# cvigilv/SimSpread.jl

Measured on AMD Instinct MI355X. Metric: predicted edges/sec + achieved HBM GB/s, W*R SpMM, higher is better.
Workload: dtype f32

## Files before the change

simspread.jl_amd/csrc/transfer.hip:

```cpp
#include <type_traits>

#include "graph.hpp"

namespace ss {

template <class T>
struct ChunkedView {
  const int* off;
  const unsigned short* idx;
  const T* val;
  int64_t rows;
};
template <class T>
static inline ChunkedView<T> view(const DevChunked<T>& m) {
  return ChunkedView<T>{m.off.p, m.idx.p, m.val.p, m.rows};
}

template <class T>
struct TransferArgs {
  int nterms;
  CsrView<T> L[2];
  const T* inv1[2];
  ChunkedView<T> M[2];
  const T* inv2;
  const int* kf;
  const int* ks;
  int64_t row_begin;
  const int* row_ids;
  int64_t nj;
  int SC;
  int nchunks;
  T* out;
  int64_t ld;
  int accumulate;
  float xmax;
  int chunk_interleave;
};
template <class T>
__device__ __forceinline__ bool chunks_in_turn(const TransferArgs<T>& p) { return p.chunk_interleave != 0; }

template <class F>
static int dispatch_bool(bool b, F&& f) {
  return b ? f(std::true_type{}) : f(std::false_type{});
}
template <int... Vs, class F>
static int dispatch_int(int v, F&& f) {
  int rc = SS_OK;
  const bool hit = ((v == Vs && ((rc = f(std::integral_constant<int, Vs>{})), true)) || ...);
  return hit ? rc : fail(SS_EINVAL, "dispatch_int: no kernel for the value %d", v);
}

template <auto Kernel, class... Args>
static int launch_lds(unsigned grid, int block, size_t lds, Args... args) {
  static std::atomic<bool> attr_done{false};
  if (!attr_done) {
    SS_HIP(hipFuncSetAttribute(reinterpret_cast<const void*>(Kernel), hipFuncAttributeMaxDynamicSharedMemorySize,
                               160 * 1024));
    attr_done = true;
  }
  hipLaunchKernelGGL(Kernel, dim3(grid), dim3(block), lds, ctx().stream, args...);
  SS_LAUNCH_CHECK();
  return SS_OK;
}

constexpr int TRANSFER_THREADS = 64;

template <class T> struct BitsOf;
template <> struct BitsOf<float> {
  static __device__ __forceinline__ float bcast(float v, int src) {
    return __int_as_float(__builtin_amdgcn_readlane(__float_as_int(v), src));
  }
  static __device__ __forceinline__ float push(int to4, float v) {
    return __int_as_float(__builtin_amdgcn_ds_permute(to4, __float_as_int(v)));
  }
  static __device__ __forceinline__ float pull(int from4, float v) {
    return __int_as_float(__builtin_amdgcn_ds_bpermute(from4, __float_as_int(v)));
  }
};
template <> struct BitsOf<double> {
  static __device__ __forceinline__ double join(int lo, int hi) {
    return __longlong_as_double(((long long)hi << 32) | (unsigned int)lo);
  }
  static __device__ __forceinline__ double bcast(double v, int src) {
    const long long b = __double_as_longlong(v);
    const int lo = __builtin_amdgcn_readlane((int)(b & 0xffffffffll), src);
    const int hi = __builtin_amdgcn_readlane((int)(b >> 32), src);
    return join(lo, hi);
  }
  static __device__ __forceinline__ double push(int to4, double v) {
    const long long b = __double_as_longlong(v);
    return join(__builtin_amdgcn_ds_permute(to4, (int)(b & 0xffffffffll)), __builtin_amdgcn_ds_permute(to4, (int)(b >> 32)));
  }
  static __device__ __forceinline__ double pull(int from4, double v) {
    const long long b = __double_as_longlong(v);
    return join(__builtin_amdgcn_ds_bpermute(from4, (int)(b & 0xffffffffll)), __builtin_amdgcn_ds_bpermute(from4, (int)(b >> 32)));
  }
};

template <class T, int U>
struct SubRows {
  int n[U];
  unsigned b[U];
  T cf[U];
  unsigned short j[U];
  T v[U];
};

template <int U, bool BINM>
__device__ __forceinline__ void subrows_load_buf(SubRows<float, U>& s, int first, int b_l, int n_l, float cf_l,
                                                 __amdgpu_buffer_rsrc_t ridx, __amdgpu_buffer_rsrc_t rval, int lane) {
#pragma unroll
  for (int u = 0; u < U; ++u) {
    const int src = first + u;
    s.b[u] = (unsigned)__builtin_amdgcn_readlane(b_l, src);
    s.n[u] = __builtin_amdgcn_readlane(n_l, src);
    s.cf[u] = BitsOf<float>::bcast(cf_l, src);
    s.j[u] = __builtin_amdgcn_raw_buffer_load_b16(ridx, lane * 2, (int)(s.b[u] * 2u), 0);
    s.v[u] = BINM ? 1.f : __builtin_bit_cast(float, __builtin_amdgcn_raw_buffer_load_b32(rval, lane * 4, (int)(s.b[u] * 4u), 0));
    __builtin_amdgcn_sched_barrier(0);
  }
}

template <class T, int U, bool BINM>
__device__ __forceinline__ void subrows_load(SubRows<T, U>& s, int first, int b_l, int n_l, T cf_l,
                                             const unsigned short* __restrict__ midx, const T* __restrict__ mval,
                                             int lane) {
#pragma unroll
  for (int u = 0; u < U; ++u) {
    const int src = first + u;
    s.b[u] = (unsigned)__builtin_amdgcn_readlane(b_l, src);
    s.n[u] = __builtin_amdgcn_readlane(n_l, src);
    s.cf[u] = BitsOf<T>::bcast(cf_l, src);
    const unsigned short* pi = midx + s.b[u];
    const T* pv = mval + s.b[u];
    s.j[u] = pi[lane];
    s.v[u] = BINM ? T(1) : pv[lane];
    __builtin_amdgcn_sched_barrier(0);
  }
}

template <class T, int U, bool DUAL>
__device__ __forceinline__ void subrows_fold(const SubRows<T, U>& s, T* __restrict__ acc, int astride, int dummy, int lane) {
  if constexpr (DUAL) {
    T* __restrict__ acc1 = acc + astride;
#pragma unroll
    for (int u = 0; u < U; u += 2) {
      const int ja = lane < s.n[u] ? (int)s.j[u] : dummy;
      const int jb = lane < s.n[u + 1] ? (int)s.j[u + 1] : dummy;
      const T ra = acc[ja], rb = acc1[jb];
      acc[ja] = fma(s.cf[u], s.v[u], ra);
      acc1[jb] = fma(s.cf[u + 1], s.v[u + 1], rb);
    }
  } else {
#pragma unroll
    for (int u = 0; u < U; ++u) {
      const int j = lane < s.n[u] ? (int)s.j[u] : dummy;
      acc[j] = fma(s.cf[u], s.v[u], acc[j]);
    }
  }
}

__device__ __forceinline__ int cvt_rpi(float x) {
  int r;
  asm("v_cvt_rpi_i32_f32 %0, %1" : "=v"(r) : "v"(x));
  return r;
}
template <int U>
__device__ __forceinline__ void subrows_fold_fixed(const SubRows<float, U>& s, unsigned* __restrict__ acc, int lane) {
#pragma unroll
  for (int u = 0; u < U; ++u) {
    const float v = lane < s.n[u] ? s.v[u] : 0.f;
    atomicAdd(&acc[s.j[u]], (unsigned)cvt_rpi(s.cf[u] * v));
  }
}

template <class T, int U, bool DUAL, bool FIX>
__device__ __forceinline__ void subrows_fold_any(const SubRows<T, U>& s, T* acc, int astride, int dummy, int lane) {
  if constexpr (FIX) subrows_fold_fixed<U>(s, reinterpret_cast<unsigned*>(acc), lane);
  else subrows_fold<T, U, DUAL>(s, acc, astride, dummy, lane);
}

template <class T, int AHEAD>
struct Tails {
  static constexpr int TAIL_AHEAD = AHEAD;
  int nt;
  int cb, cn;
  T ccf;
  unsigned short tj[TAIL_AHEAD];
  T tv[TAIL_AHEAD];
};

template <class T, int TAIL_AHEAD, class LD>
__device__ __forceinline__ void tails_fetch(Tails<T, TAIL_AHEAD>& t, int r0, int lane, LD&& ld) {
#pragma unroll
  for (int i = 0; i < TAIL_AHEAD; ++i) {
    if (4 * (r0 + i) >= t.nt) break;
    const unsigned b = (unsigned)__builtin_amdgcn_ds_bpermute((4 * (r0 + i) + (lane >> 4)) * 4, t.cb);
    ld(b + 64u + (unsigned)(lane & 15), t.tj[i], t.tv[i]);
    __builtin_amdgcn_sched_barrier(0);
  }
}

template <class T, int TAIL_AHEAD, class LD>
__device__ __forceinline__ void tails_begin(Tails<T, TAIL_AHEAD>& t, int b_l, int n_l, T cf_l, int lane, LD&& ld) {
  const unsigned long long longs = __ballot(n_l > 64);
  t.nt = __builtin_popcountll(longs);
  if (t.nt == 0) return;
  const int k = (int)__builtin_amdgcn_mbcnt_hi((unsigned)(longs >> 32), __builtin_amdgcn_mbcnt_lo((unsigned)longs, 0u));
  const int to4 = (n_l > 64 ? k : t.nt + lane - k) * 4;
  t.cb = __builtin_amdgcn_ds_permute(to4, b_l);
  t.cn = __builtin_amdgcn_ds_permute(to4, n_l);
  t.ccf = BitsOf<T>::push(to4, cf_l);
  tails_fetch(t, 0, lane, ld);
}

template <class T, bool BINM, bool FIX, int TAIL_AHEAD, class LD>
__device__ __forceinline__ void tails_finish(Tails<T, TAIL_AHEAD>& t, int b_l, int n_l, T cf_l, T* __restrict__ acc, int dummy,
                                             const unsigned short* __restrict__ midx, const T* __restrict__ mval, int lane,
                                             LD&& ld) {
  if (t.nt == 0) return;
  for (int r0 = 0; 4 * r0 < t.nt; r0 += TAIL_AHEAD) {
    if (r0 > 0) tails_fetch(t, r0, lane, ld);
#pragma unroll
    for (int i = 0; i < TAIL_AHEAD; ++i) {
      if (4 * (r0 + i) >= t.nt) break;
      const int from4 = (4 * (r0 + i) + (lane >> 4)) * 4;
      const int tn = __builtin_amdgcn_ds_bpermute(from4, t.cn) - 64;
      const T tcf = BitsOf<T>::pull(from4, t.ccf);
      const bool live = (lane & 15) < tn;
      if constexpr (FIX) {
        atomicAdd(reinterpret_cast<unsigned*>(acc) + (live ? (int)t.tj[i] : dummy),
                  (unsigned)cvt_rpi(live ? (float)(tcf * t.tv[i]) : 0.f));
      } else {
#pragma unroll
        for (int g = 0; g < 4; ++g) {
          const int j = (live && (lane >> 4) == g) ? (int)t.tj[i] : dummy;
          acc[j] = fma(tcf, t.tv[i], acc[j]);
        }
      }
    }
  }
  unsigned long long m = __ballot(n_l > 80);
  while (m != 0ull) {
    const int src = __builtin_ctzll(m);
    m &= m - 1ull;
    const int n = __builtin_amdgcn_readlane(n_l, src);
    const unsigned b = (unsigned)__builtin_amdgcn_readlane(b_l, src);
    const T cf = BitsOf<T>::bcast(cf_l, src);
    for (int x = 80 + lane; x < n; x += 64) {
      const int j = midx[b + x];
      const T v = BINM ? T(1) : mval[b + x];
      if constexpr (FIX) atomicAdd(reinterpret_cast<unsigned*>(acc) + j, (unsigned)cvt_rpi((float)(cf * v)));
      else acc[j] = fma(cf, v, acc[j]);
    }
  }
}

struct FixedScale {
  float scale, unscale;
};
template <class F>
__device__ __forceinline__ FixedScale fixed_scale(int lb, int le, int lane, float xmax, F&& abs_coef) {
  float sabs = 0.f;
  for (int q = lb + lane; q < le; q += 64) sabs += abs_coef(q);
#pragma unroll
  for (int o = 32; o > 0; o >>= 1) sabs += __shfl_xor(sabs, o);
  int e = 0;
  (void)frexpf(sabs * xmax, &e);
  if (!(sabs * xmax > 0.f)) e = 0;
  e = e < -90 ? -90 : (e > 120 ? 120 : e);
  return FixedScale{ldexpf(1.f, 30 - e), ldexpf(1.f, e - 30)};
}

template <class T, bool LOO, int U, bool BINM, bool DUAL, bool FIX = false, bool BUF = false>
__global__ void __launch_bounds__(TRANSFER_THREADS) transfer_kernel(TransferArgs<T> p) {
  static_assert(64 % (2 * U) == 0, "U must divide 32");
  extern __shared__ __align__(16) unsigned char smem_raw[];
  T* acc = reinterpret_cast<T*>(smem_raw);
  const int astride = p.SC + 64;
  constexpr int NCOPY = DUAL ? 2 : 1;
  unsigned* bits = reinterpret_cast<unsigned*>(acc + NCOPY * astride);
  const int lane = threadIdx.x;
  int c;
  int64_t r;
  if (p.nchunks > 8 && p.nchunks % 8 == 0 && !chunks_in_turn(p)) {
    const int64_t nrows = (int64_t)gridDim.x / p.nchunks, per = nrows * 8;
    const int64_t grp = blockIdx.x / per, rem = blockIdx.x - grp * per;
    r = rem >> 3;
    c = (int)(grp * 8 + (rem & 7));
  } else {
    c = blockIdx.x % p.nchunks;
    r = blockIdx.x / p.nchunks;
  }
  const int64_t gr = p.row_ids ? (int64_t)p.row_ids[p.row_begin + r] : p.row_begin + r;
  const int64_t j0 = (int64_t)c * p.SC;
  const int jn = (int)((p.nj - j0 < p.SC) ? (p.nj - j0) : p.SC);
  const int dummy = p.SC + lane;

  for (int j = lane; j < NCOPY * astride; j += 64) acc[j] = T(0);
  if (LOO)
    for (int j = lane; j < (p.SC + 31) / 32; j += 64) bits[j] = 0u;
  __syncthreads();

  float fix_unscale = 1.f;
  for (int t = 0; t < p.nterms; ++t) {
    const CsrView<T> L = p.L[t];
    const ChunkedView<T> M = p.M[t];
    const int* __restrict__ off = M.off + (int64_t)c * M.rows;
    const unsigned short* __restrict__ midx = M.idx;
    const T* __restrict__ mval = M.val;
    const int lb = L.ptr[gr], le = L.ptr[gr + 1];
    float scale = 1.f;
    if constexpr (FIX) {
      float sabs = 0.f;
      for (int q = lb + lane; q < le; q += 64) sabs += fabsf((float)(L.val[q] * p.inv1[t][L.idx[q]]));
#pragma unroll
      for (int o = 32; o > 0; o >>= 1) sabs += __shfl_xor(sabs, o);
      int e = 0;
      (void)frexpf(sabs * p.xmax, &e);
      if (!(sabs * p.xmax > 0.f)) e = 0;
      e = e < -90 ? -90 : (e > 120 ? 120 : e);
      scale = ldexpf(1.f, 30 - e);
      fix_unscale = ldexpf(1.f, e - 30);
    }
    for (int g0 = lb; g0 < le; g0 += 64) {
      const int q = g0 + lane;
      int b_l = 0, n_l = 0;
      T cf_l = T(0);
      if (q < le) {
        const int a = L.idx[q];
        const T lv = L.val[q];
        if (LOO) {
          const int d = p.kf[a] - 1;
          cf_l = (a != (int)gr && d > 0) ? lv * (T(1) / T(d)) : T(0);
        } else {
          cf_l = lv * p.inv1[t][a];
          if constexpr (FIX) cf_l = (T)((float)cf_l * scale);
        }
        if (cf_l != T(0)) { b_l = off[a]; n_l = off[a + 1] - b_l; }
      }
      const int cnt = __builtin_amdgcn_readfirstlane((le - g0 < 64) ? (le - g0) : 64);
      SubRows<T, U> A, B;
      auto load = [&](SubRows<T, U>& sr, int first) __attribute__((always_inline)) {
        if constexpr (BUF) {
          const __amdgpu_buffer_rsrc_t ridx = __builtin_amdgcn_make_buffer_rsrc((void*)midx, 0, -1, 0x00020000);
          const __amdgpu_buffer_rsrc_t rval = __builtin_amdgcn_make_buffer_rsrc((void*)mval, 0, -1, 0x00020000);
          subrows_load_buf<U, BINM>(sr, first, b_l, n_l, cf_l, ridx, rval, lane);
        } else {
          subrows_load<T, U, BINM>(sr, first, b_l, n_l, cf_l, midx, mval, lane);
        }
      };
      auto tail_ld = [&](unsigned e, unsigned short& j, T& v) __attribute__((always_inline)) {
        if constexpr (BUF) {
          const __amdgpu_buffer_rsrc_t ridx = __builtin_amdgcn_make_buffer_rsrc((void*)midx, 0, -1, 0x00020000);
          const __amdgpu_buffer_rsrc_t rval = __builtin_amdgcn_make_buffer_rsrc((void*)mval, 0, -1, 0x00020000);
          j = __builtin_amdgcn_raw_buffer_load_b16(ridx, (int)(e * 2u), 0, 0);
          v = BINM ? 1.f : __builtin_bit_cast(float, __builtin_amdgcn_raw_buffer_load_b32(rval, (int)(e * 4u), 0, 0));
        } else {
          j = midx[e];
          v = BINM ? T(1) : mval[e];
        }
      };
      Tails<T, (BINM ? 4 : 2)> tails;
      tails_begin(tails, b_l, n_l, cf_l, lane, tail_ld);
      load(A, 0);
      for (int u0 = 0; u0 < cnt; u0 += 2 * U) {
        if (u0 + U < cnt) load(B, u0 + U);
        subrows_fold_any<T, U, DUAL, FIX>(A, acc, astride, dummy, lane);
        if (u0 + U < cnt) {
          if (u0 + 2 * U < cnt) load(A, u0 + 2 * U);
          subrows_fold_any<T, U, DUAL, FIX>(B, acc, astride, dummy, lane);
        }
      }
      tails_finish<T, BINM, FIX>(tails, b_l, n_l, cf_l, acc, dummy, midx, mval, lane, tail_ld);
    }
  }
  if (LOO) {
    const ChunkedView<T> M = p.M[0];
    const int* off = M.off + (int64_t)c * M.rows;
    for (int x = off[gr] + lane; x < off[gr + 1]; x += 64) {
      const int j = M.idx[x];
      atomicOr(&bits[j >> 5], 1u << (j & 31));
    }
  }
  __syncthreads();

  T* orow = p.out + r * p.ld + j0;
  for (int j = lane; j < jn; j += 64) {
    T z;
    T sum = DUAL ? acc[j] + acc[astride + j] : acc[j];
    if constexpr (FIX) sum = (T)((float)reinterpret_cast<const int*>(acc)[j] * fix_unscale);
    if (LOO) {
      const int d = p.ks[j0 + j] - (int)((bits[j >> 5] >> (j & 31)) & 1u);
      z = (d > 0 && (j0 + j) != gr) ? sum * (T(1) / T(d)) : T(0);
    } else {
      z = sum * p.inv2[j0 + j];
      if (p.accumulate) z += orow[j];
    }
    orow[j] = z;
  }
}

constexpr int TRANSFER_U = 8;

static bool transfer_dual() { return env_int("SS_TRANSFER_DUAL", 0) != 0; }

static int transfer_u() {
  const int u = (int)env_int("SS_TRANSFER_U", TRANSFER_U);
  return (u == 4 || u == 16) ? u : 8;
}

template <class T>
__global__ void transfer_coef_kernel(const int* __restrict__ ptr, const int* __restrict__ idx, const T* __restrict__ val,
                                     const T* __restrict__ inv1, int64_t row_begin, int64_t nrows, T* __restrict__ coef) {
  const int lo = ptr[row_begin], hi = ptr[row_begin + nrows];
  for (int64_t e = (int64_t)lo + (int64_t)blockIdx.x * blockDim.x + threadIdx.x; e < hi; e += (int64_t)gridDim.x * blockDim.x)
    coef[e] = val[e] * inv1[idx[e]];
}

enum { TB_PLAIN, TB_QFLAT, TB_WIDE, TB_WIDE2 };
constexpr int WIDE_META = 64 * 12;
constexpr int WIDE_LIST = 64;
constexpr int W2_TBL = 64 * 12;
template <int KIND, class T>
struct BlockLayout {
  static constexpr bool EXACT = KIND != TB_PLAIN;
  static constexpr int shared_bytes = KIND == TB_WIDE ? 64 : 0;
  __host__ __device__ static int64_t offs_bytes(int64_t mrows) { return (((mrows + 1) * 4 + 15) / 16) * 16; }
  __host__ __device__ static int64_t lens_bytes(int64_t mrows) { return EXACT ? ((mrows * 2 + 15) / 16) * 16 : 0; }
  __host__ __device__ static int acc_elems(int SC) { return SC + 64; }
  __host__ __device__ static int acc_bytes(int SC) {
    return KIND == TB_WIDE || KIND == TB_WIDE2 ? (((SC + 4) * 4 + 15) / 16) * 16 : acc_elems(SC) * (int)sizeof(T);
  }
  __host__ __device__ static int per_wave(int SC) {
    return acc_bytes(SC) + (KIND == TB_WIDE ? WIDE_META + WIDE_LIST : KIND == TB_WIDE2 ? 2 * W2_TBL + 4 * 64 : 0);
  }
  __device__ static unsigned char* wave_base(unsigned char* smem, int offs_b, int lens_b, int wave, int SC) {
    return smem + offs_b + lens_b + shared_bytes + (size_t)wave * (size_t)per_wave(SC);
  }
};

struct BlockWave {
  int lane, c, jn, lb, le;
  int64_t r, gr, j0;
};

template <bool EXACT, class T, class A>
__device__ __forceinline__ bool block_prologue(BlockWave& w, const TransferArgs<T>& p, int64_t nrows, int wave, int* offs,
                                               unsigned short* lens, const unsigned short* glen, A* acc, int nacc) {
  const int nw = blockDim.x >> 6;
  w.lane = threadIdx.x & 63;
  w.c = blockIdx.x % p.nchunks;
  w.r = (int64_t)(blockIdx.x / p.nchunks) * nw + wave;
  const ChunkedView<T> M = p.M[0];
  {
    const int* __restrict__ off = M.off + (int64_t)w.c * M.rows;
    for (int64_t i = threadIdx.x; i <= M.rows; i += blockDim.x) offs[i] = off[i];
    if constexpr (EXACT) {
      const unsigned short* __restrict__ gl = glen + (int64_t)w.c * M.rows;
      for (int64_t i = threadIdx.x; i < M.rows; i += blockDim.x) lens[i] = gl[i];
    }
  }
  for (int j = w.lane; j < nacc; j += 64) acc[j] = A(0);
  __syncthreads();
  return w.r < nrows;
}
template <class T>
__device__ __forceinline__ void block_row(BlockWave& w, const TransferArgs<T>& p) {
  w.gr = p.row_begin + w.r;
  w.j0 = (int64_t)w.c * p.SC;
  w.jn = (int)((p.nj - w.j0 < p.SC) ? (p.nj - w.j0) : p.SC);
  const int* lptr = p.L[0].ptr;
  w.lb = __builtin_amdgcn_readfirstlane(lptr[w.gr]);
  w.le = __builtin_amdgcn_readfirstlane(lptr[w.gr + 1]);
}

template <class T>
__device__ __forceinline__ void fixed_store(const TransferArgs<T>& p, int64_t r, int64_t j0, int jn, int lane, const void* acc,
                                            float unscale) {
  T* orow = p.out + r * p.ld + j0;
  const int* iacc = reinterpret_cast<const int*>(acc);
  for (int j = lane; j < jn; j += 64) orow[j] = (T)((float)iacc[j] * unscale) * p.inv2[j0 + j];
}

typedef float f4 __attribute__((ext_vector_type(4)));
typedef unsigned u2 __attribute__((ext_vector_type(2)));

template <bool BINM>
__device__ __forceinline__ void quad_fetch(const u2* midx4, const f4* mval4, int quad, float cfv, int rem, u2& oj, f4& ov,
                                           float& ocf) {
  ocf = cfv;
  oj = midx4[quad];
  if constexpr (BINM) ov = f4{rem > 0 ? 1.f : 0.f, rem > 1 ? 1.f : 0.f, rem > 2 ? 1.f : 0.f, rem > 3 ? 1.f : 0.f};
  else ov = mval4[quad];
}
__device__ __forceinline__ void quad_fold(unsigned* acc, u2 j, f4 v, float cf) {
  atomicAdd(acc + (j.x & 0xffffu), (unsigned)cvt_rpi(cf * v.x));
  atomicAdd(acc + (j.x >> 16), (unsigned)cvt_rpi(cf * v.y));
  atomicAdd(acc + (j.y & 0xffffu), (unsigned)cvt_rpi(cf * v.z));
  atomicAdd(acc + (j.y >> 16), (unsigned)cvt_rpi(cf * v.w));
}

__device__ __forceinline__ void raw_load(const int* lidx, const float* coef, int lb, int le, int lane, int g, int& a, float& cf) {
  const int q = lb + g * 64 + lane;
  a = 0;
  cf = 0.f;
  if (q < le) { a = lidx[q]; cf = coef[q]; }
}

template <class T, int U, bool BINM, bool FIX>
__global__ void __launch_bounds__(1024) transfer_block_kernel(TransferArgs<T> p, const T* __restrict__ coef, int64_t nrows,
                                                              int align, int offs_bytes, float xmax) {
  using Lay = BlockLayout<TB_PLAIN, T>;
  extern __shared__ __align__(16) unsigned char smem_raw[];
  int* offs = reinterpret_cast<int*>(smem_raw);
  const int wave = threadIdx.x >> 6;
  const int astride = p.SC + 64;
  T* acc = reinterpret_cast<T*>(smem_raw + offs_bytes) + (size_t)wave * Lay::acc_elems(p.SC);
  BlockWave w;
  if (!block_prologue<false>(w, p, nrows, wave, offs, nullptr, nullptr, acc, astride)) return;
  w.gr = p.row_begin + w.r;
  w.j0 = (int64_t)w.c * p.SC;
  w.jn = (int)((p.nj - w.j0 < p.SC) ? (p.nj - w.j0) : p.SC);
  const int lane = w.lane, lb = p.L[0].ptr[w.gr], le = p.L[0].ptr[w.gr + 1];
  const int dummy = p.SC + lane;
  const CsrView<T> L = p.L[0];
  const unsigned short* __restrict__ midx = p.M[0].idx;
  const T* __restrict__ mval = p.M[0].val;
  float scale = 1.f, unscale = 1.f;
  if constexpr (FIX) {
    const FixedScale fs = fixed_scale(lb, le, lane, xmax, [&](int q) __attribute__((always_inline)) { return fabsf((float)coef[q]); });
    scale = fs.scale;
    unscale = fs.unscale;
  }
  for (int g0 = lb; g0 < le; g0 += 64) {
    const int q = g0 + lane;
    int b_l = 0, n_l = 0;
    T cf_l = T(0);
    if (q < le) {
      const int a = L.idx[q];
      cf_l = coef[q];
      if constexpr (FIX) cf_l = (T)((float)cf_l * scale);
      if (cf_l != T(0)) {
        const int o0 = offs[a], o1 = offs[a + 1];
        b_l = o0 * align;
        n_l = (o1 - o0) * align;
      }
    }
    const int cnt = __builtin_amdgcn_readfirstlane((le - g0 < 64) ? (le - g0) : 64);
    SubRows<T, U> A, B;
    auto load = [&](SubRows<T, U>& sr, int first) __attribute__((always_inline)) {
      subrows_load<T, U, BINM>(sr, first, b_l, n_l, cf_l, midx, mval, lane);
    };
    auto tail_ld = [&](unsigned e, unsigned short& j, T& v) __attribute__((always_inline)) {
      j = midx[e];
      v = BINM ? T(1) : mval[e];
    };
    Tails<T, (BINM ? 4 : 2)> tails;
    tails_begin(tails, b_l, n_l, cf_l, lane, tail_ld);
    load(A, 0);
    for (int u0 = 0; u0 < cnt; u0 += 2 * U) {
      if (u0 + U < cnt) load(B, u0 + U);
      subrows_fold_any<T, U, false, FIX>(A, acc, astride, dummy, lane);
      if (u0 + U < cnt) {
        if (u0 + 2 * U < cnt) load(A, u0 + 2 * U);
        subrows_fold_any<T, U, false, FIX>(B, acc, astride, dummy, lane);
      }
    }
    tails_finish<T, BINM, FIX>(tails, b_l, n_l, cf_l, acc, dummy, midx, mval, lane, tail_ld);
  }
  if constexpr (FIX) {
    fixed_store(p, w.r, w.j0, w.jn, lane, acc, unscale);
  } else {
    T* orow = p.out + w.r * p.ld + w.j0;
    for (int j = lane; j < w.jn; j += 64) orow[j] = acc[j] * p.inv2[w.j0 + j];
  }
}

template <class T, int D, bool BINM>
__global__ void __launch_bounds__(1024) transfer_qflat_kernel(TransferArgs<T> p, const T* __restrict__ coef, int64_t nrows,
                                                             int align, int offs_bytes, int lens_bytes, float xmax,
                                                             const unsigned short* __restrict__ glen) {
  static_assert(std::is_same<T, float>::value, "fixed-point sums: fp32 graphs only");
  extern __shared__ __align__(16) unsigned char smem_raw[];
  int* offs = reinterpret_cast<int*>(smem_raw);
  unsigned short* lens = reinterpret_cast<unsigned short*>(smem_raw + offs_bytes);
  const int lane = threadIdx.x & 63;
  const int wave = __builtin_amdgcn_readfirstlane(threadIdx.x >> 6);
  const int astride = p.SC + 64;
  unsigned* acc = reinterpret_cast<unsigned*>(BlockLayout<TB_QFLAT, T>::wave_base(smem_raw, offs_bytes, lens_bytes, wave, p.SC));
  BlockWave w;
  if (!block_prologue<true>(w, p, nrows, wave, offs, lens, glen, acc, astride)) return;
  block_row(w, p);
  const ChunkedView<T> M = p.M[0];
  const CsrView<T> L = p.L[0];
  const int64_t r = w.r, j0 = w.j0;
  const int jn = w.jn, lb = w.lb, le = w.le;
  const unsigned short* __restrict__ midx = M.idx;
  const T* __restrict__ mval = M.val;
  float scale, unscale;
  {
    float sabs = 0.f;
    for (int q = lb + lane; q < le; q += 64) sabs += fabsf(coef[q]);
#pragma unroll
    for (int o = 32; o > 0; o >>= 1) sabs += __shfl_xor(sabs, o);
    int e = 0;
    (void)frexpf(sabs * xmax, &e);
    if (!(sabs * xmax > 0.f)) e = 0;
    e = e < -90 ? -90 : (e > 120 ? 120 : e);
    scale = ldexpf(1.f, 30 - e);
    unscale = ldexpf(1.f, e - 30);
  }
  const int ngroups = (le - lb + 63) >> 6;
  auto raw_load = [&](int g, int& a, float& cf) __attribute__((always_inline)) {
    const int q = lb + g * 64 + lane;
    a = 0;
    cf = 0.f;
    if (q < le) { a = L.idx[q]; cf = coef[q]; }
  };
  auto meta = [&](int a, float cf, int& b_l, int& n_l, float& cf_l) __attribute__((always_inline)) {
    cf_l = cf * scale;
    b_l = 0;
    n_l = 0;
    if (cf_l != 0.f) {
      b_l = (offs[a] * align) >> 2;
      n_l = ((int)lens[a] + 3) >> 2;
    }
  };
  int Pc = 0, dc = 0, ra, bn, nn;
  float cc = 0.f, cn, rc;
  int total = 0, nst = 0, t = 0, gcur = -1;
  raw_load(0, ra, rc); meta(ra, rc, bn, nn, cn);
  raw_load(1, ra, rc);
  bool done = false;
  auto switch_group = [&]() __attribute__((always_inline)) {
    ++gcur;
    int incl = nn;
#pragma unroll
    for (int o = 1; o < 64; o <<= 1) {
      const int up = __shfl_up(incl, o);
      if (lane >= o) incl += up;
    }
    Pc = incl - nn;
    dc = bn - Pc;
    cc = cn;
    total = __builtin_amdgcn_readlane(incl, 63);
    nst = (total + 63) >> 6;
    t = 0;
    meta(ra, rc, bn, nn, cn);
    raw_load(gcur + 2, ra, rc);
  };
  u2 sj[D];
  f4 sv[D];
  float sc[D];
  const f4* __restrict__ mval4 = reinterpret_cast<const f4*>(mval);
  const u2* __restrict__ midx4 = reinterpret_cast<const u2*>(midx);
  auto next_step = [&](u2& oj, f4& ov, float& ocf) __attribute__((always_inline)) {
    if (t >= nst) {
      if (gcur + 1 < ngroups) switch_group();
      else done = true;
    }
    float cfv = 0.f;
    int addr = lane;
    if (t < nst) {
      const int lo = t << 6;
      const int pos = lo + lane;
      const unsigned long long le_mask = __ballot(Pc <= lo);
      const int own0 = __builtin_popcountll(le_mask) - 1;
      unsigned long long m = __ballot(Pc > lo && Pc <= lo + 63);
      cfv = __int_as_float(__builtin_amdgcn_readlane(__float_as_int(cc), own0));
      int dlv = __builtin_amdgcn_readlane(dc, own0);
      while (m != 0ull) {
        const int i = __builtin_ctzll(m);
        m &= m - 1ull;
        const int Pi = __builtin_amdgcn_readlane(Pc, i);
        const float cfi = __int_as_float(__builtin_amdgcn_readlane(__float_as_int(cc), i));
        const int dli = __builtin_amdgcn_readlane(dc, i);
        const bool in = pos >= Pi;
        cfv = in ? cfi : cfv;
        dlv = in ? dli : dlv;
      }
      const bool valid = pos < total;
      cfv = valid ? cfv : 0.f;
      addr = valid ? pos + dlv : lane;
      ++t;
    }
    quad_fetch<BINM>(midx4, mval4, addr, cfv, 4, oj, ov, ocf);
  };
#pragma unroll
  for (int i = 0; i < D; ++i) next_step(sj[i], sv[i], sc[i]);
  while (!done) {
#pragma unroll
    for (int i = 0; i < D; ++i) {
      quad_fold(acc, sj[i], sv[i], sc[i]);
      next_step(sj[i], sv[i], sc[i]);
    }
  }
#pragma unroll
  for (int i = 0; i < D; ++i) quad_fold(acc, sj[i], sv[i], sc[i]);
  fixed_store(p, r, j0, jn, lane, acc, unscale);
}

template <int D, bool BINM>
__global__ void __launch_bounds__(1024) transfer_wide_kernel(TransferArgs<float> p, const float* __restrict__ coef,
                                                             int64_t nrows, int align, int offs_bytes, int lens_bytes,
                                                             float xmax, const unsigned short* __restrict__ glen) {
  extern __shared__ __align__(16) unsigned char smem_raw[];
  int* offs = reinterpret_cast<int*>(smem_raw);
  unsigned short* lens = reinterpret_cast<unsigned short*>(smem_raw + offs_bytes);
  unsigned char* ident = smem_raw + offs_bytes + lens_bytes;
  const int lane = threadIdx.x & 63, nw = blockDim.x >> 6;
  const int wave = __builtin_amdgcn_readfirstlane(threadIdx.x >> 6);
  using Lay = BlockLayout<TB_WIDE, float>;
  const int accb = Lay::acc_bytes(p.SC);
  unsigned char* mine = Lay::wave_base(smem_raw, offs_bytes, lens_bytes, wave, p.SC);
  unsigned* acc = reinterpret_cast<unsigned*>(mine);
  unsigned char* metab = mine + accb;
  unsigned char* list = metab + WIDE_META;
  const int c = blockIdx.x % p.nchunks;
  const int64_t r = (int64_t)(blockIdx.x / p.nchunks) * nw + wave;
  const ChunkedView<float> M = p.M[0];
  const CsrView<float> L = p.L[0];
  {
    const int* __restrict__ off = M.off + (int64_t)c * M.rows;
    const unsigned short* __restrict__ gl = glen + (int64_t)c * M.rows;
    for (int64_t i = threadIdx.x; i <= M.rows; i += blockDim.x) offs[i] = off[i];
    for (int64_t i = threadIdx.x; i < M.rows; i += blockDim.x) lens[i] = gl[i];
    if (threadIdx.x < 64) ident[threadIdx.x] = (unsigned char)threadIdx.x;
  }
  for (int j = lane; j < p.SC; j += 64) acc[j] = 0u;
  __syncthreads();
  if (r >= nrows) return;
  const int64_t gr = p.row_begin + r;
  const int64_t j0 = (int64_t)c * p.SC;
  const int jn = (int)((p.nj - j0 < p.SC) ? (p.nj - j0) : p.SC);
  const int lb = __builtin_amdgcn_readfirstlane(L.ptr[gr]), le = __builtin_amdgcn_readfirstlane(L.ptr[gr + 1]);
  const FixedScale fs = fixed_scale(lb, le, lane, xmax, [&](int q) __attribute__((always_inline)) { return fabsf(coef[q]); });
  const float scale = fs.scale, unscale = fs.unscale;
  const int ngroups = (le - lb + 63) >> 6;
  const f4* __restrict__ mval4 = reinterpret_cast<const f4*>(M.val);
  const u2* __restrict__ midx4 = reinterpret_cast<const u2*>(M.idx);
  int gcur = -1, level = 0, st = 0, nst = 0, nlist = 0, qoff = 0;
  int ncur = 0;
  int ra;
  float rc;
  raw_load(L.idx, coef, lb, le, lane, 0, ra, rc);
  bool done = false;
  auto open_group = [&]() __attribute__((always_inline)) {
    ++gcur;
    const float cf = rc * scale;
    int b = 0, n = 0;
    if (cf != 0.f) { b = (offs[ra] * align) >> 2; n = (int)lens[ra]; }
    raw_load(L.idx, coef, lb, le, lane, gcur + 1, ra, rc);
    ncur = n;
    unsigned* m = reinterpret_cast<unsigned*>(metab + lane * 12);
    m[0] = (unsigned)b; m[1] = (unsigned)n; m[2] = __float_as_uint(cf);
    level = 0;
    st = 0;
    qoff = 0;
    const int cnt = (le - lb - gcur * 64 < 64) ? (le - lb - gcur * 64) : 64;
    nlist = cnt;
    nst = (cnt + 3) >> 2;
  };
  auto next_level = [&]() __attribute__((always_inline)) {
    const int covered = 64 + 16 * level;
    ++level;
    qoff = covered >> 2;
    const bool more = ncur > covered;
    const unsigned long long mk = __ballot(more);
    nlist = __builtin_popcountll(mk);
    if (more) list[__builtin_amdgcn_mbcnt_hi((unsigned)(mk >> 32), __builtin_amdgcn_mbcnt_lo((unsigned)mk, 0u))] = (unsigned char)lane;
    st = 0;
    nst = (nlist + 15) >> 4;
  };
  u2 sj[D];
  f4 sv[D];
  float sc[D];
  auto next_step = [&](u2& oj, f4& ov, float& ocf) __attribute__((always_inline)) {
    if (st >= nst) {
      if (gcur >= 0 && nlist > 0) next_level();
      else if (gcur + 1 < ngroups) open_group();
      else done = true;
    }
    float cfv = 0.f;
    int quad = lane;
    int rem = 0;
    if (st < nst) {
      const int sh = level == 0 ? 4 : 2;
      const int pos = (st << (6 - sh)) + (lane >> sh);
      const int e = lane & ((1 << sh) - 1);
      const unsigned char* lst = level == 0 ? ident : list;
      const int fi = pos < nlist ? (int)lst[pos] : 0;
      const unsigned* m = reinterpret_cast<const unsigned*>(metab + fi * 12);
      const int b = (int)m[0], n = (int)m[1];
      const float cf = __uint_as_float(m[2]);
      const int qe = qoff + e;
      const bool valid = pos < nlist && 4 * qe < n;
      cfv = valid ? cf : 0.f;
      quad = valid ? b + qe : lane;
      rem = n - 4 * qe;
      ++st;
    }
    quad_fetch<BINM>(midx4, mval4, quad, cfv, rem, oj, ov, ocf);
  };
#pragma unroll
  for (int i = 0; i < D; ++i) next_step(sj[i], sv[i], sc[i]);
  while (!done) {
#pragma unroll
    for (int i = 0; i < D; ++i) {
      quad_fold(acc, sj[i], sv[i], sc[i]);
      next_step(sj[i], sv[i], sc[i]);
    }
  }
#pragma unroll
  for (int i = 0; i < D; ++i) quad_fold(acc, sj[i], sv[i], sc[i]);
  float* orow = p.out + r * p.ld + j0;
  const int* iacc = reinterpret_cast<const int*>(acc);
  for (int j = lane; j < jn; j += 64) orow[j] = ((float)iacc[j] * unscale) * p.inv2[j0 + j];
}

constexpr int W2_STEPS = 20;
constexpr int W2_D = 4;
template <bool BINM>
__global__ void __launch_bounds__(1024) transfer_wide2_kernel(TransferArgs<float> p, const float* __restrict__ coef,
                                                              int64_t nrows, int align, int offs_bytes, int lens_bytes,
                                                              float xmax, const unsigned short* __restrict__ glen) {
  extern __shared__ __align__(16) unsigned char smem_raw[];
  int* offs = reinterpret_cast<int*>(smem_raw);
  unsigned short* lens = reinterpret_cast<unsigned short*>(smem_raw + offs_bytes);
  const int lane = threadIdx.x & 63, nw = blockDim.x >> 6;
  const int wave = __builtin_amdgcn_readfirstlane(threadIdx.x >> 6);
  using Lay = BlockLayout<TB_WIDE2, float>;
  const int accb = Lay::acc_bytes(p.SC);
  unsigned char* mine = Lay::wave_base(smem_raw, offs_bytes, lens_bytes, wave, p.SC);
  unsigned* acc = reinterpret_cast<unsigned*>(mine);
  unsigned char* tbl0 = mine + accb;
  unsigned char* lst0 = tbl0 + 2 * W2_TBL;
  const int c = blockIdx.x % p.nchunks;
  const int64_t r = (int64_t)(blockIdx.x / p.nchunks) * nw + wave;
  const ChunkedView<float> M = p.M[0];
  const CsrView<float> L = p.L[0];
  {
    const int* __restrict__ off = M.off + (int64_t)c * M.rows;
    const unsigned short* __restrict__ gl = glen + (int64_t)c * M.rows;
    for (int64_t i = threadIdx.x; i <= M.rows; i += blockDim.x) offs[i] = off[i];
    for (int64_t i = threadIdx.x; i < M.rows; i += blockDim.x) lens[i] = gl[i];
  }
  for (int j = lane; j < p.SC; j += 64) acc[j] = 0u;
  __syncthreads();
  if (r >= nrows) return;
  const int64_t gr = p.row_begin + r;
  const int64_t j0 = (int64_t)c * p.SC;
  const int jn = (int)((p.nj - j0 < p.SC) ? (p.nj - j0) : p.SC);
  const int lb = __builtin_amdgcn_readfirstlane(L.ptr[gr]), le = __builtin_amdgcn_readfirstlane(L.ptr[gr + 1]);
  const FixedScale fs = fixed_scale(lb, le, lane, xmax, [&](int q) __attribute__((always_inline)) { return fabsf(coef[q]); });
  const float scale = fs.scale, unscale = fs.unscale;
  const int ngroups = (le - lb + 63) >> 6;
  const f4* __restrict__ mval4 = reinterpret_cast<const f4*>(M.val);
  const u2* __restrict__ midx4 = reinterpret_cast<const u2*>(M.idx);
  const unsigned short* __restrict__ midx = M.idx;
  const float* __restrict__ mval = M.val;
  const int lastq = le > lb ? le - 1 : lb;
  auto raw_load = [&](int g, int& a, float& cf) __attribute__((always_inline)) {
    const int q = lb + g * 64 + lane;
    const int qc = q < le ? q : lastq;
    a = L.idx[qc];
    const float x = coef[qc];
    cf = q < le ? x : 0.f;
  };
  int ra = 0;
  float rc = 0.f;
  auto open_group = [&](int g) __attribute__((always_inline)) {
    unsigned char* tb = tbl0 + (g & 1) * W2_TBL;
    unsigned char* l1 = lst0 + (g & 1) * 128;
    unsigned char* l2 = l1 + 64;
    const float cf = (g < ngroups) ? rc * scale : 0.f;
    int b = 0, n = 0;
    if (cf != 0.f) { b = (offs[ra] * align) >> 2; n = (int)lens[ra]; }
    raw_load(g + 1, ra, rc);
    unsigned* m = reinterpret_cast<unsigned*>(tb + lane * 12);
    m[0] = (unsigned)b; m[1] = (unsigned)n; m[2] = __float_as_uint(cf);
    const unsigned long long m1 = __ballot(n > 64);
    const int r1 = __builtin_amdgcn_mbcnt_hi((unsigned)(m1 >> 32), __builtin_amdgcn_mbcnt_lo((unsigned)m1, 0u));
    const bool in1 = n > 64 && r1 < 48;
    const unsigned long long m2 = __ballot(in1 && n > 80);
    const int r2 = __builtin_amdgcn_mbcnt_hi((unsigned)(m2 >> 32), __builtin_amdgcn_mbcnt_lo((unsigned)m2, 0u));
    const bool in2 = in1 && n > 80 && r2 < 16;
    l1[lane] = 255; l2[lane] = 255;
    if (in1) l1[r1] = (unsigned char)lane;
    if (in2) l2[r2] = (unsigned char)lane;
    const int cov = in2 ? 96 : (in1 ? 80 : 64);
    if (__ballot(n > cov) != 0ull) {
      for (int x = cov; x < n; ++x) {
        const int at = 4 * b + x;
        atomicAdd(acc + midx[at], (unsigned)cvt_rpi(cf * (BINM ? 1.f : mval[at])));
      }
    }
  };
  u2 sj[W2_D];
  f4 sv[W2_D];
  float sc[W2_D];
  auto gen = [&](int s, int par, u2& oj, f4& ov, float& ocf) __attribute__((always_inline)) {
    const unsigned char* tb = tbl0 + par * W2_TBL;
    int fi, e, qoff;
    bool have = true;
    if (s < 16) {
      fi = 4 * s + (lane >> 4);
      e = lane & 15;
      qoff = 0;
    } else {
      const unsigned char* lst = lst0 + par * 128 + (s < 19 ? 0 : 64);
      const int pos = (s < 19 ? 16 * (s - 16) : 0) + (lane >> 2);
      fi = (int)lst[pos];
      have = fi != 255;
      fi = have ? fi : 0;
      e = lane & 3;
      qoff = s < 19 ? 16 : 20;
    }
    const unsigned* m = reinterpret_cast<const unsigned*>(tb + fi * 12);
    const int b = (int)m[0], n = (int)m[1];
    const float cf = __uint_as_float(m[2]);
    const int qe = qoff + e;
    const bool valid = have && 4 * qe < n;
    quad_fetch<BINM>(midx4, mval4, valid ? b + qe : lane, valid ? cf : 0.f, n - 4 * qe, oj, ov, ocf);
  };
  if (ngroups > 0) {
    raw_load(0, ra, rc);
    open_group(0);
#pragma unroll
    for (int i = 0; i < W2_D; ++i) gen(i, 0, sj[i], sv[i], sc[i]);
    for (int g = 0; g < ngroups; ++g) {
      const int par = g & 1;
#pragma unroll
      for (int s = 0; s < W2_STEPS; ++s) {
        if (s == W2_STEPS - W2_D) open_group(g + 1);
        quad_fold(acc, sj[s % W2_D], sv[s % W2_D], sc[s % W2_D]);
        if (s + W2_D < W2_STEPS) gen(s + W2_D, par, sj[s % W2_D], sv[s % W2_D], sc[s % W2_D]);
        else gen(s + W2_D - W2_STEPS, par ^ 1, sj[s % W2_D], sv[s % W2_D], sc[s % W2_D]);
      }
    }
  }
  fixed_store(p, r, j0, jn, lane, acc, unscale);
}

template <int KIND, class T>
static int transfer_block_waves(int64_t mrows, int SC) {
  using Lay = BlockLayout<KIND, T>;
  const int64_t fixed_bytes = Lay::offs_bytes(mrows) + Lay::lens_bytes(mrows) + Lay::shared_bytes;
  const int64_t room = (int64_t)ctx().lds_per_block - fixed_bytes;
  int64_t nw = room > 0 ? room / Lay::per_wave(SC) : 0;
  if (nw > 16) nw = 16;
  nw = env_int_in("SS_TRANSFER_NW", 1, nw, nw);
  return nw >= 8 ? (int)nw : 0;
}

template <class T>
bool transfer_block_fits(int64_t mrows, int SC) {
  return transfer_block_waves<TB_PLAIN, T>(mrows, SC) > 0;
}

template <int KIND, auto Kernel, class T>
static int launch_block_kernel(const TransferArgs<T>& p, const DevChunked<T>& Mt, const T* coef, int64_t nrows, int nw,
                               float xmax) {
  using Lay = BlockLayout<KIND, T>;
  const int offs_bytes = (int)Lay::offs_bytes(Mt.rows), lens_bytes = (int)Lay::lens_bytes(Mt.rows);
  const unsigned grid = (unsigned)(ceil_div(nrows, (int64_t)nw) * p.nchunks);
  const size_t lds = (size_t)offs_bytes + (size_t)lens_bytes + Lay::shared_bytes + (size_t)nw * (size_t)Lay::per_wave(p.SC);
  if constexpr (Lay::EXACT)
    return launch_lds<Kernel>(grid, 64 * nw, lds, p, coef, nrows, Mt.align, offs_bytes, lens_bytes, xmax,
                              (const unsigned short*)Mt.len.p);
  else
    return launch_lds<Kernel>(grid, 64 * nw, lds, p, coef, nrows, Mt.align, offs_bytes, xmax);
}

template <class T>
int launch_transfer_block(const DevCsr<T>& L, const T* inv1, const DevChunked<T>& Mt, const T* inv2, int64_t row_begin,
                          int64_t nrows, int64_t nj, T* out, int64_t ld, T* coef, float xmax, bool fixed) {
  if (nrows <= 0 || nj <= 0) return SS_OK;
  const int nw = transfer_block_waves<TB_PLAIN, T>(Mt.rows, Mt.SC);
  if (nw == 0) return fail(SS_EUNSUPPORTED, "transfer_block: offsets + accumulators do not fit in LDS");
  TransferArgs<T> p{};
  p.nterms = 1;
  p.L[0] = view(L);
  p.M[0] = view(Mt);
  p.inv2 = inv2;
  p.row_begin = row_begin;
  p.nj = nj;
  p.SC = Mt.SC;
  p.nchunks = Mt.nchunks;
  p.out = out;
  p.ld = ld;
  if (ceil_div(nrows, (int64_t)nw) * p.nchunks >= (1LL << 31))
    return fail(SS_EUNSUPPORTED, "transfer grid too large; lower SS_TRANSFER_BYTES");
  path_add("transfer_block");
  hipLaunchKernelGGL(transfer_coef_kernel<T>, dim3(grid_1d(L.nnz > 0 ? L.nnz : 1, 256, 256 * 8)), dim3(256), 0, ctx().stream,
                     L.ptr.p, L.idx.p, L.val.p, inv1, row_begin, nrows, coef);
  SS_LAUNCH_CHECK();
  constexpr bool CANFIX = std::is_same<T, float>::value;
  const bool fx = CANFIX && fixed;
  if (fx) path_add("fixed_point");
  const bool binm = Mt.binary;
  if constexpr (CANFIX) {
    const int wide2 = (int)env_int("SS_TRANSFER_WIDE2", 0), wide = (int)env_int("SS_TRANSFER_WIDE", 0),
              qflat = (int)env_int("SS_TRANSFER_QFLAT", 0);
    if ((wide2 > 0 || wide > 0 || qflat > 0) && fixed && Mt.align == 32 && Mt.len_ok) {
      if (wide2 > 0) {
        if (const int n = transfer_block_waves<TB_WIDE2, T>(Mt.rows, Mt.SC)) {
          path_add("wide2");
          return dispatch_bool(binm, [&](auto B) {
            return launch_block_kernel<TB_WIDE2, transfer_wide2_kernel<decltype(B)::value>>(p, Mt, coef, nrows, n, xmax);
          });
        }
      } else if (wide > 0) {
        if (const int n = transfer_block_waves<TB_WIDE, T>(Mt.rows, Mt.SC)) {
          path_add("wide");
          return dispatch_int<2, 4>(wide == 2 ? 2 : 4, [&](auto D) {
            return dispatch_bool(binm, [&](auto B) {
              return launch_block_kernel<TB_WIDE, transfer_wide_kernel<decltype(D)::value, decltype(B)::value>>(
                  p, Mt, coef, nrows, n, xmax);
            });
          });
        }
      } else if (const int n = transfer_block_waves<TB_QFLAT, T>(Mt.rows, Mt.SC)) {
        path_add("qflat");
        return dispatch_bool(binm, [&](auto B) {
          return launch_block_kernel<TB_QFLAT, transfer_qflat_kernel<float, 4, decltype(B)::value>>(p, Mt, coef, nrows, n, xmax);
        });
      }
    }
  }
  return dispatch_int<4, 8>(transfer_u() == 4 ? 4 : 8, [&](auto U) {
    return dispatch_bool(binm, [&](auto B) {
      return dispatch_bool(fx, [&](auto F) {
        constexpr bool FIX = CANFIX && decltype(F)::value;
        return launch_block_kernel<TB_PLAIN, transfer_block_kernel<T, decltype(U)::value, decltype(B)::value, FIX>>(
            p, Mt, coef, nrows, nw, xmax);
      });
    });
  });
}

template <class T, bool LOO>
static int launch_transfer_variant(const TransferArgs<T>& p, unsigned grid, size_t lds, bool binm, bool dual) {
  auto launch = [&](auto kernel) {
    hipLaunchKernelGGL(kernel, dim3(grid), dim3(TRANSFER_THREADS), lds, ctx().stream, p);
    SS_LAUNCH_CHECK();
    return (int)SS_OK;
  };
  const int u = transfer_u();
  if constexpr (std::is_same<T, float>::value && !LOO) {
    const bool buf = !dual && env_int("SS_TRANSFER_LD", 0) == 1;
    const bool fix = !dual && env_int("SS_TRANSFER_FIX1", 0) == 1 && p.nterms == 1 && !p.accumulate;
    if (buf) path_add("buffer_loads");
    if (fix) path_add("fixed_point");
    if (buf || fix)
      return dispatch_int<4, 8>(u == 4 ? 4 : 8, [&](auto U) {
        return dispatch_bool(binm, [&](auto B) {
          return dispatch_bool(fix, [&](auto F) {
            return dispatch_bool(buf, [&](auto BF) {
              return launch(transfer_kernel<T, LOO, decltype(U)::value, decltype(B)::value, false, decltype(F)::value,
                                            decltype(BF)::value>);
            });
          });
        });
      });
  }
  return dispatch_int<4, 8, 16>(u, [&](auto U) {
    return dispatch_bool(binm, [&](auto B) {
      return dispatch_bool(dual, [&](auto D) {
        return launch(transfer_kernel<T, LOO, decltype(U)::value, decltype(B)::value, decltype(D)::value>);
      });
    });
  });
}

template <class T>
int launch_transfer(int nterms, const DevCsr<T>* L[2], const T* inv1[2], const DevChunked<T>* Mt[2],
                    const T* inv2, int64_t row_begin, int64_t nrows, int64_t nj, T* out, int64_t ld,
                    const int* row_ids, bool accumulate) {
  if (nrows <= 0 || nj <= 0) return SS_OK;
  TransferArgs<T> p{};
  p.nterms = nterms;
  for (int t = 0; t < nterms; ++t) {
    p.L[t] = view(*L[t]);
    p.M[t] = view(*Mt[t]);
    p.inv1[t] = inv1[t];
    if (Mt[t]->SC != Mt[0]->SC || Mt[t]->nchunks != Mt[0]->nchunks)
      return fail(SS_EINVAL, "transfer operands were cut with different chunk sizes");
  }
  p.inv2 = inv2;
  p.row_begin = row_begin;
  p.row_ids = row_ids;
  p.nj = nj;
  p.SC = Mt[0]->SC;
  p.nchunks = Mt[0]->nchunks;
  p.out = out;
  p.ld = ld;
  p.accumulate = accumulate ? 1 : 0;
  p.xmax = 1.0f;
  p.chunk_interleave = env_off("SS_TRANSFER_ORDER") ? 1 : 0;
  bool binm = true;
  for (int t = 0; t < nterms; ++t) binm = binm && Mt[t]->binary;
  const int64_t grid = nrows * p.nchunks;
  if (grid >= (1LL << 31)) return fail(SS_EUNSUPPORTED, "transfer grid too large; lower SS_TRANSFER_BYTES");
  const bool dual = transfer_dual();
  path_add("transfer");
  const size_t lds = (size_t)(p.SC + 64) * sizeof(T) * (dual ? 2 : 1);
  return launch_transfer_variant<T, false>(p, (unsigned)grid, lds, binm, dual);
}

template <class T>
int launch_transfer_loo(const DevCsr<T>& X, const DevChunked<T>& XT, const int* kf, const int* ks,
                        int64_t i_begin, int64_t nrows, T* out, int64_t ld) {
  if (nrows <= 0) return SS_OK;
  TransferArgs<T> p{};
  p.nterms = 1;
  p.L[0] = view(X);
  p.M[0] = view(XT);
  p.kf = kf;
  p.ks = ks;
  p.row_begin = i_begin;
  p.nj = X.rows;
  p.SC = XT.SC;
  p.nchunks = XT.nchunks;
  p.out = out;
  p.ld = ld;
  p.chunk_interleave = env_off("SS_TRANSFER_ORDER") ? 1 : 0;
  const int64_t grid = nrows * p.nchunks;
  if (grid >= (1LL << 31)) return fail(SS_EUNSUPPORTED, "transfer grid too large; lower SS_TRANSFER_BYTES");
  const bool dual = transfer_dual();
  path_add("transfer_loo");
  const size_t lds = (size_t)(p.SC + 64) * sizeof(T) * (dual ? 2 : 1) + (size_t)((p.SC + 31) / 32) * 4;
  return launch_transfer_variant<T, true>(p, (unsigned)grid, lds, XT.binary, dual);
}

#define SS_INSTANTIATE(T)                                                                                   \
  template int launch_transfer<T>(int, const DevCsr<T>*[2], const T*[2], const DevChunked<T>*[2], const T*, \
                                  int64_t, int64_t, int64_t, T*, int64_t, const int*, bool);                      \
  template int launch_transfer_block<T>(const DevCsr<T>&, const T*, const DevChunked<T>&, const T*, int64_t, int64_t, \
                                        int64_t, T*, int64_t, T*, float, bool);                               \
  template bool transfer_block_fits<T>(int64_t, int);                                                        \
  template int launch_transfer_loo<T>(const DevCsr<T>&, const DevChunked<T>&, const int*, const int*,       \
                                      int64_t, int64_t, T*, int64_t);
SS_INSTANTIATE(float)
SS_INSTANTIATE(double)

}
```

Before: 51.92 billion.

## Prefetch next neighbour group's indices and metadata during current fold

Software-pipelines the per-group gather of L indices/values and the dependent inv1/offset lookups. The next 64-neighbour group is fetched before the fold loop and its metadata after it, so the dependent-load latency overlaps with accumulation work instead of stalling at the start of each group. The first group's neighbour load is also issued before the accumulator zeroing and barrier. This adds register pressure and some redundant clamped loads for the last group, which could lower occupancy.

Measured after the change: 52.26 billion (median of 4 runs). Within noise of the previous version (+0.7%).

```diff
diff --git a/simspread.jl_amd/csrc/transfer.hip b/simspread.jl_amd/csrc/transfer.hip
--- a/simspread.jl_amd/csrc/transfer.hip
+++ b/simspread.jl_amd/csrc/transfer.hip
@@ -297,6 +297,24 @@
   const int jn = (int)((p.nj - j0 < p.SC) ? (p.nj - j0) : p.SC);
   const int dummy = p.SC + lane;
 
+  auto nbr_fetch = [&](const CsrView<T>& L, int g0, int le, int& a, T& lv) __attribute__((always_inline)) {
+    const int q = g0 + lane;
+    const int qc = q < le ? q : le - 1;
+    a = L.idx[qc];
+    lv = L.val[qc];
+  };
+  auto meta_fetch = [&](const T* __restrict__ inv1, const int* __restrict__ off, int a, T& inv, int& kf, int& o0, int& o1)
+                        __attribute__((always_inline)) {
+    if (LOO) kf = p.kf[a];
+    else inv = inv1[a];
+    o0 = off[a];
+    o1 = off[a + 1];
+  };
+  int lb = __builtin_amdgcn_readfirstlane(p.L[0].ptr[gr]), le = __builtin_amdgcn_readfirstlane(p.L[0].ptr[gr + 1]);
+  int a_c = 0;
+  T lv_c = T(0);
+  if (lb < le) nbr_fetch(p.L[0], lb, le, a_c, lv_c);
+
   for (int j = lane; j < NCOPY * astride; j += 64) acc[j] = T(0);
   if (LOO)
     for (int j = lane; j < (p.SC + 31) / 32; j += 64) bits[j] = 0u;
@@ -309,7 +327,15 @@
     const int* __restrict__ off = M.off + (int64_t)c * M.rows;
     const unsigned short* __restrict__ midx = M.idx;
     const T* __restrict__ mval = M.val;
-    const int lb = L.ptr[gr], le = L.ptr[gr + 1];
+    const T* __restrict__ inv1 = p.inv1[t];
+    if (t > 0) {
+      lb = __builtin_amdgcn_readfirstlane(L.ptr[gr]);
+      le = __builtin_amdgcn_readfirstlane(L.ptr[gr + 1]);
+      if (lb < le) nbr_fetch(L, lb, le, a_c, lv_c);
+    }
+    T inv_c = T(0);
+    int kf_c = 0, o0_c = 0, o1_c = 0;
+    if (lb < le) meta_fetch(inv1, off, a_c, inv_c, kf_c, o0_c, o1_c);
     float scale = 1.f;
     if constexpr (FIX) {
       float sabs = 0.f;
@@ -325,20 +351,17 @@
     }
     for (int g0 = lb; g0 < le; g0 += 64) {
       const int q = g0 + lane;
-      int b_l = 0, n_l = 0;
-      T cf_l = T(0);
-      if (q < le) {
-        const int a = L.idx[q];
-        const T lv = L.val[q];
-        if (LOO) {
-          const int d = p.kf[a] - 1;
-          cf_l = (a != (int)gr && d > 0) ? lv * (T(1) / T(d)) : T(0);
-        } else {
-          cf_l = lv * p.inv1[t][a];
-          if constexpr (FIX) cf_l = (T)((float)cf_l * scale);
-        }
-        if (cf_l != T(0)) { b_l = off[a]; n_l = off[a + 1] - b_l; }
+      T cf_l;
+      if (LOO) {
+        const int d = kf_c - 1;
+        cf_l = (a_c != (int)gr && d > 0) ? lv_c * (T(1) / T(d)) : T(0);
+      } else {
+        cf_l = lv_c * inv_c;
+        if constexpr (FIX) cf_l = (T)((float)cf_l * scale);
       }
+      cf_l = q < le ? cf_l : T(0);
+      const int b_l = cf_l != T(0) ? o0_c : 0;
+      const int n_l = cf_l != T(0) ? o1_c - o0_c : 0;
       const int cnt = __builtin_amdgcn_readfirstlane((le - g0 < 64) ? (le - g0) : 64);
       SubRows<T, U> A, B;
       auto load = [&](SubRows<T, U>& sr, int first) __attribute__((always_inline)) {
@@ -364,6 +387,9 @@
       Tails<T, (BINM ? 4 : 2)> tails;
       tails_begin(tails, b_l, n_l, cf_l, lane, tail_ld);
       load(A, 0);
+      int a_n;
+      T lv_n;
+      nbr_fetch(L, g0 + 64, le, a_n, lv_n);
       for (int u0 = 0; u0 < cnt; u0 += 2 * U) {
         if (u0 + U < cnt) load(B, u0 + U);
         subrows_fold_any<T, U, DUAL, FIX>(A, acc, astride, dummy, lane);
@@ -372,7 +398,16 @@
           subrows_fold_any<T, U, DUAL, FIX>(B, acc, astride, dummy, lane);
         }
       }
+      T inv_n = T(0);
+      int kf_n = 0, o0_n, o1_n;
+      meta_fetch(inv1, off, a_n, inv_n, kf_n, o0_n, o1_n);
       tails_finish<T, BINM, FIX>(tails, b_l, n_l, cf_l, acc, dummy, midx, mval, lane, tail_ld);
+      a_c = a_n;
+      lv_c = lv_n;
+      inv_c = inv_n;
+      kf_c = kf_n;
+      o0_c = o0_n;
+      o1_c = o1_n;
     }
   }
   if (LOO) {
```
